# JacobYoung115/VisualSLAM

Hardware: AMD Instinct MI355X
Metric: frames/sec @1080p (Harris + DoG keypoint detection) (higher is better)
Workload: dtype u8

## Files before the change

### visualslam_amd/csrc/kernels_compact.hip.h

```cpp
#pragma once
#include <hip/hip_runtime.h>

#include "kernels_generic.hip.h"
#include "kernels_harris_strip.hip.h"

namespace vslam {

constexpr int CMP_CHUNK = 256;

__device__ __forceinline__ int select64(unsigned long long w, unsigned int k) {
    unsigned int x = (unsigned int)w;
    int pos = 0;
    unsigned int c = __popc(x);
    if (k >= c) k -= c, pos = 32, x = (unsigned int)(w >> 32);
#pragma unroll
    for (int s = 16; s >= 1; s >>= 1) {
        c = __popc(x & ((1u << s) - 1u));
        if (k >= c) k -= c, pos += s, x >>= s;
    }
    return pos;
}

struct HarrisStripEntries {
    static constexpr int WORDS = 4;
    struct Info {
        int row, c0;
    };
    const unsigned long long* flags;
    size_t fframe;
    int rows, cols, nstrips;
    const float* resp;
    size_t rframe;
    vslam_kp* out;
    __device__ size_t count() const { return (size_t)rows * nstrips; }
    __device__ unsigned int load(int f, size_t e, unsigned long long (&w)[4]) const {
        const unsigned long long* F = flags + f * fframe + e * 4;
#pragma unroll
        for (int k = 0; k < 4; ++k) w[k] = F[k];
        return __popcll(w[0]) + __popcll(w[1]) + __popcll(w[2]) + __popcll(w[3]);
    }
    __device__ Info info(int, size_t e) const {
        const int r = (int)((unsigned int)e / (unsigned int)nstrips), strip = (int)((unsigned int)e % (unsigned int)nstrips);
        return Info{r, strip * HS_STRIP_W - 8};
    }
    __device__ void emit(int f, const Info& in, const unsigned long long (&w)[4], unsigned int k, size_t slot) const {
        int l = 0;
#pragma unroll
        for (int s = 32; s >= 1; s >>= 1) {
            const unsigned long long m = (1ull << (l + s)) - 1ull;
            const unsigned int c = __popcll(w[0] & m) + __popcll(w[1] & m) + __popcll(w[2] & m) + __popcll(w[3] & m);
            if (c <= k) l += s;
        }
        const unsigned long long m = (1ull << l) - 1ull;
        k -= __popcll(w[0] & m) + __popcll(w[1] & m) + __popcll(w[2] & m) + __popcll(w[3] & m);
        const unsigned int nib = (unsigned int)((w[0] >> l) & 1ull) | ((unsigned int)((w[1] >> l) & 1ull) << 1) |
                                 ((unsigned int)((w[2] >> l) & 1ull) << 2) | ((unsigned int)((w[3] >> l) & 1ull) << 3);
        unsigned int x = nib;
        for (unsigned int i = 0; i < k; ++i) x &= x - 1;
        const int c = in.c0 + 4 * l + (__ffs((int)x) - 1);
        vslam_kp kp;
        kp.row = in.row;
        kp.col = c;
        kp.response = resp[f * rframe + (size_t)in.row * cols + c];
        out[slot] = kp;
    }
};

struct DogEntries {
    static constexpr int WORDS = 1;
    struct Info {
        int octave, level, i, j0, step;
        unsigned int row_off;
    };
    const unsigned long long* lflags;
    size_t bframe;
    const uint8_t* pyr;
    size_t pframe;
    ExtGeom g;
    int o_begin, o_end;
    vslam_point* out;
    __device__ size_t first() const { return g.bits_off[o_begin]; }
    __device__ size_t count() const {
        return g.bits_off[o_end - 1] + (size_t)3 * g.lat_rows[o_end - 1] * g.wpr[o_end - 1] - g.bits_off[o_begin];
    }
    __device__ unsigned int load(int f, size_t e, unsigned long long (&w)[4]) const {
        w[0] = lflags[f * bframe + first() + e];
        return __popcll(w[0]);
    }
    __device__ Info info(int, size_t e) const {
        const size_t wi = first() + e;
        int o = o_begin;
        while (o + 1 < o_end && wi >= g.bits_off[o + 1]) ++o;
        const unsigned int wl = (unsigned int)(wi - g.bits_off[o]);
        const unsigned int wpr = g.wpr[o], lr = g.lat_rows[o];
        const int level = (int)(wl / (lr * wpr)) + 1;
        const int li = (int)((wl / wpr) % lr), lj0 = (int)(wl % wpr) * 64;
        const size_t P = (size_t)g.rows[o] * g.pitch[o];
        const int i = g.pad + li * g.window;
        return Info{o, level, i, g.pad + lj0 * g.window, g.window,
                    (unsigned int)(g.oct_off[o] + (size_t)(VSLAM_NUM_LEVELS + level) * P + (size_t)(i - g.pad) * g.pitch[o])};
    }
    __device__ void emit(int f, const Info& in, const unsigned long long (&w)[4], unsigned int k, size_t slot) const {
        const int j = in.j0 + select64(w[0], k) * in.step;
        vslam_point pt;
        pt.row = in.i;
        pt.col = j;
        pt.value = pyr[f * pframe + in.row_off + (j - g.pad)];
        if (g.localize) {
            const int o = in.octave;
            const size_t P = (size_t)g.rows[o] * g.pitch[o];
            const uint8_t* dog = pyr + f * pframe + g.oct_off[o] + (size_t)VSLAM_NUM_LEVELS * P;
            int d_x, d_y, d_s, nv;
            dog_differences(dog, P, g.rows[o], g.cols[o], g.pitch[o], g.pad, in.level, in.i, j, d_x, d_y, d_s);
            feature_point_localization(d_x, d_y, d_s, pt.value, nv, g.loc_lut);
            pt.value = nv;
        }
        pt.padding = g.pad;
        pt.octave = in.octave;
        pt.level = in.level;
        out[slot] = pt;
    }
};

struct OrientEntries {
    static constexpr int WORDS = 1;
    struct Info {
        int row, col, octave, level;
    };
    const unsigned long long* masks;
    const vslam_point* kps;
    size_t n;
    vslam_point* out;
    __device__ size_t count() const { return n; }
    __device__ unsigned int load(int, size_t e, unsigned long long (&w)[4]) const {
        w[0] = masks[e];
        return __popcll(w[0]);
    }
    __device__ Info info(int, size_t e) const {
        const vslam_point kp = kps[e];
        return Info{kp.row, kp.col, kp.octave, kp.level};
    }
    __device__ void emit(int, const Info& in, const unsigned long long (&w)[4], unsigned int k, size_t slot) const {
        vslam_point pt;
        pt.row = in.row;
        pt.col = in.col;
        pt.value = select64(w[0], k) * 10;
        pt.padding = 0;
        pt.octave = in.octave;
        pt.level = in.level;
        out[slot] = pt;
    }
};

struct SurvivorEntries {
    static constexpr int WORDS = 1;
    struct Info {
        unsigned int first;
    };
    const unsigned long long* flags;
    size_t fwords;
    unsigned int* surv;
    __device__ size_t count() const { return fwords; }
    __device__ unsigned int load(int f, size_t e, unsigned long long (&w)[4]) const {
        w[0] = flags[f * fwords + e];
        return __popcll(w[0]);
    }
    __device__ Info info(int, size_t e) const { return Info{(unsigned int)(e * 64)}; }
    __device__ void emit(int, const Info& in, const unsigned long long (&w)[4], unsigned int k, size_t slot) const {
        surv[slot] = in.first + (unsigned int)select64(w[0], k);
    }
};

struct OrientBatchEntries {
    static constexpr int WORDS = 1;
    struct Info {
        int row, col, octave, level;
    };
    const unsigned long long* masks;
    const unsigned int* surv;
    const unsigned int* scounts;
    unsigned int scap;
    const vslam_point* pts;
    unsigned int pcap;
    vslam_point* out;
    __device__ size_t count() const { return scap; }
    __device__ unsigned int load(int f, size_t e, unsigned long long (&w)[4]) const {
        w[0] = e < min(scounts[f], scap) ? masks[(size_t)f * scap + e] : 0ull;
        return __popcll(w[0]);
    }
    __device__ Info info(int f, size_t e) const {
        const vslam_point kp = pts[(size_t)f * pcap + surv[(size_t)f * scap + e]];
        return Info{kp.row, kp.col, kp.octave, kp.level};
    }
    __device__ void emit(int, const Info& in, const unsigned long long (&w)[4], unsigned int k, size_t slot) const {
        vslam_point pt;
        pt.row = in.row;
        pt.col = in.col;
        pt.value = select64(w[0], k) * 10;
        pt.padding = 0;
        pt.octave = in.octave;
        pt.level = in.level;
        out[slot] = pt;
    }
};

struct MatchEntries {
    static constexpr int WORDS = 1;
    struct Info {
        unsigned int first;
    };
    const unsigned long long* flags;
    size_t fwords;
    const vslam_nn2* nn;
    unsigned int qcap;
    vslam_match* out;
    __device__ size_t count() const { return fwords; }
    __device__ unsigned int load(int f, size_t e, unsigned long long (&w)[4]) const {
        w[0] = flags[f * fwords + e];
        return __popcll(w[0]);
    }
    __device__ Info info(int, size_t e) const { return Info{(unsigned int)(e * 64)}; }
    __device__ void emit(int f, const Info& in, const unsigned long long (&w)[4], unsigned int k, size_t slot) const {
        const unsigned int q = in.first + (unsigned int)select64(w[0], k);
        const vslam_nn2 r = nn[(size_t)f * qcap + q];
        vslam_match m;
        m.query = (int)q;
        m.train = r.index;
        m.dist2 = r.dist2;
        out[slot] = m;
    }
};

struct EpipolarEntries {
    static constexpr int WORDS = 1;
    struct Info {
        unsigned int first;
    };
    const unsigned long long* flags;
    size_t fwords;
    const vslam_match* matches;
    const unsigned int* counts;
    unsigned int mcap;
    vslam_match* out;
    __device__ size_t count() const { return fwords; }
    __device__ unsigned int load(int f, size_t e, unsigned long long (&w)[4]) const {
        w[0] = e * 64 < min(counts[f], mcap) ? flags[f * fwords + e] : 0ull;
        return __popcll(w[0]);
    }
    __device__ Info info(int, size_t e) const { return Info{(unsigned int)(e * 64)}; }
    __device__ void emit(int f, const Info& in, const unsigned long long (&w)[4], unsigned int k, size_t slot) const {
        out[slot] = matches[(size_t)f * mcap + in.first + (unsigned int)select64(w[0], k)];
    }
};

__device__ __forceinline__ unsigned int block_excl_scan_256(unsigned int v, unsigned int* wsum, unsigned int& total) {
    const int lane = threadIdx.x & 63, wave = threadIdx.x >> 6;
    unsigned int inc = v;
    for (int off = 1; off < 64; off <<= 1) {
        const unsigned int t = __shfl_up(inc, off);
        if (lane >= off) inc += t;
    }
    if (lane == 63) wsum[wave] = inc;
    __syncthreads();
    unsigned int base = 0, tot = 0;
#pragma unroll
    for (int w = 0; w < 4; ++w) {
        const unsigned int s = wsum[w];
        if (w < wave) base += s;
        tot += s;
    }
    total = tot;
    return base + inc - v;
}

template <class E>
__global__ __launch_bounds__(256) void k_flag_count(const E ent, unsigned int* __restrict__ chunk_tot, int nchunks) {
    __shared__ unsigned int wsum[4];
    const int f = blockIdx.z;
    const size_t e = (size_t)blockIdx.x * CMP_CHUNK + threadIdx.x;
    unsigned long long w[4] = {0, 0, 0, 0};
    const unsigned int cnt = e < ent.count() ? ent.load(f, e, w) : 0u;
    unsigned int total;
    block_excl_scan_256(cnt, wsum, total);
    if (threadIdx.x == 0) chunk_tot[(size_t)f * nchunks + blockIdx.x] = total;
}

__global__ __launch_bounds__(256) void k_chunk_scan(unsigned int* __restrict__ chunk_tot, int nchunks,
                                                     unsigned int* __restrict__ counts, int append) {
    __shared__ unsigned int wsum[4];
    const int f = blockIdx.x;
    unsigned int* T = chunk_tot + (size_t)f * nchunks;
    unsigned int running = append ? counts[f] : 0u;
    for (int base = 0; base < nchunks; base += 256) {
        const int i = base + threadIdx.x;
        const unsigned int v = i < nchunks ? T[i] : 0u;
        unsigned int total;
        const unsigned int ex = block_excl_scan_256(v, wsum, total);
        if (i < nchunks) T[i] = running + ex;
        running += total;
        __syncthreads();
    }
    if (threadIdx.x == 0) counts[f] = running;
}

template <class E>
__global__ __launch_bounds__(256) void k_flag_scatter(const E ent, const unsigned int* __restrict__ chunk_off, int nchunks,
                                                       unsigned int cap) {
    __shared__ unsigned int wsum[4];
    __shared__ unsigned int s_ex[CMP_CHUNK];
    __shared__ unsigned long long s_w[E::WORDS][CMP_CHUNK];
    __shared__ typename E::Info s_info[CMP_CHUNK];
    const int f = blockIdx.z, t = threadIdx.x;
    const size_t e = (size_t)blockIdx.x * CMP_CHUNK + t;
    unsigned long long w[4] = {0, 0, 0, 0};
    const unsigned int cnt = e < ent.count() ? ent.load(f, e, w) : 0u;
    unsigned int total;
    s_ex[t] = block_excl_scan_256(cnt, wsum, total);
#pragma unroll
    for (int k = 0; k < E::WORDS; ++k) s_w[k][t] = w[k];
    if (cnt) s_info[t] = ent.info(f, e);
    __syncthreads();
    const unsigned int base = chunk_off[(size_t)f * nchunks + blockIdx.x];
    if (base >= cap) return;
    for (unsigned int r = t; r < total; r += CMP_CHUNK) {
        if (base + r >= cap) break;
        int lo = 0;
#pragma unroll
        for (int s = CMP_CHUNK / 2; s >= 1; s >>= 1)
            if (s_ex[lo + s] <= r) lo += s;
        unsigned long long we[4] = {0, 0, 0, 0};
#pragma unroll
        for (int k = 0; k < E::WORDS; ++k) we[k] = s_w[k][lo];
        ent.emit(f, s_info[lo], we, r - s_ex[lo], (size_t)f * cap + base + r);
    }
}

__global__ __launch_bounds__(256) void k_pack_offsets(const unsigned int* __restrict__ counts, unsigned int cap, int n,
                                                       unsigned long long* __restrict__ offsets) {
    __shared__ unsigned long long sc[256];
    const int t = threadIdx.x;
    unsigned long long running = 0;
    for (int base = 0; base < n; base += 256) {
        const int i = base + t;
        const unsigned long long v = i < n ? (unsigned long long)min(counts[i], cap) : 0ull;
        sc[t] = v;
        __syncthreads();
        for (int off = 1; off < 256; off <<= 1) {
            const unsigned long long a = t >= off ? sc[t - off] : 0ull;
            __syncthreads();
            sc[t] += a;
            __syncthreads();
        }
        if (i < n) offsets[i] = running + sc[t] - v;
        running += sc[255];
        __syncthreads();
    }
    if (t == 0) offsets[n] = running;
}

__global__ __launch_bounds__(256) void k_pack_copy(const unsigned int* __restrict__ lists, unsigned int rec_dw, unsigned int cap,
                                                    const unsigned int* __restrict__ counts,
                                                    const unsigned long long* __restrict__ offsets,
                                                    unsigned int* __restrict__ packed, unsigned long long packed_dw) {
    const int f = blockIdx.z;
    const unsigned long long ndw = (unsigned long long)min(counts[f], cap) * rec_dw;
    const unsigned int* src = lists + (size_t)f * cap * rec_dw;
    const unsigned long long d0 = offsets[f] * rec_dw;
    for (unsigned long long i = (unsigned long long)blockIdx.x * 256 + threadIdx.x; i < ndw; i += (unsigned long long)gridDim.x * 256)
        if (d0 + i < packed_dw) packed[d0 + i] = src[i];
}

__global__ __launch_bounds__(256) void k_pack_points16(const int2* __restrict__ lists, unsigned int cap, const unsigned int* __restrict__ counts,
                                                        const unsigned long long* __restrict__ offsets, uint4* __restrict__ packed,
                                                        unsigned long long packed_recs) {
    const int f = blockIdx.z;
    const unsigned int nrec = min(counts[f], cap);
    const int2* src = lists + (size_t)f * cap * 3;
    const unsigned long long d0 = offsets[f];
    for (unsigned int i = blockIdx.x * 256 + threadIdx.x; i < nrec; i += gridDim.x * 256) {
        const int2 a = src[3 * (size_t)i], b = src[3 * (size_t)i + 1], c = src[3 * (size_t)i + 2];
        if (d0 + i < packed_recs)
            packed[d0 + i] = make_uint4((unsigned int)a.x, (unsigned int)a.y, (unsigned int)b.x,
                                        ((unsigned int)c.y & 0xffu) | (((unsigned int)c.x & 0xffu) << 8) | (((unsigned int)b.y & 0xffffu) << 16));
    }
}

__global__ __launch_bounds__(256) void k_count_totals(const unsigned int* __restrict__ a, const unsigned int* __restrict__ b, int n,
                                                       unsigned long long* __restrict__ totals) {
    __shared__ unsigned long long sa[4], sb[4];
    unsigned long long ta = 0, tb = 0;
    for (int i = threadIdx.x; i < n; i += 256) {
        if (a) ta += a[i];
        if (b) tb += b[i];
    }
    for (int off = 32; off >= 1; off >>= 1) {
        ta += __shfl_down(ta, off);
        tb += __shfl_down(tb, off);
    }
    if ((threadIdx.x & 63) == 0) sa[threadIdx.x >> 6] = ta, sb[threadIdx.x >> 6] = tb;
    __syncthreads();
    if (threadIdx.x == 0) {
        totals[0] = sa[0] + sa[1] + sa[2] + sa[3];
        totals[1] = sb[0] + sb[1] + sb[2] + sb[3];
    }
}

}
```

### visualslam_amd/csrc/kernels_harris_strip.hip.h

```cpp
#pragma once
#include <hip/hip_runtime.h>

#include <type_traits>

#include "kernels_generic.hip.h"
#include "vslam_harris_launch.h"

namespace vslam {

typedef short s2_t __attribute__((ext_vector_type(2)));

__device__ __forceinline__ uint32_t pk_sub_i16(uint32_t a, uint32_t b) {
    return __builtin_bit_cast(uint32_t, (s2_t)(__builtin_bit_cast(s2_t, a) - __builtin_bit_cast(s2_t, b)));
}
struct HarrisStripArgs {
    const uint8_t* img;
    size_t frame;
    int rows, cols;
    float k;
    float* resp;
    uint8_t* mask;
    float* nms2;
    unsigned long long* flags;
    size_t fframe;
    int nstrips, seg;
    uint8_t* dump;
};

__device__ __forceinline__ uint32_t dpp_left(uint32_t v) { return (uint32_t)__builtin_amdgcn_mov_dpp((int)v, 0x138, 0xf, 0xf, true); }
__device__ __forceinline__ uint32_t dpp_right(uint32_t v) { return (uint32_t)__builtin_amdgcn_mov_dpp((int)v, 0x130, 0xf, 0xf, true); }
__device__ __forceinline__ float dpp_left_f(float v) { return __uint_as_float(dpp_left(__float_as_uint(v))); }
__device__ __forceinline__ float dpp_right_f(float v) { return __uint_as_float(dpp_right(__float_as_uint(v))); }
__device__ __forceinline__ float max3f(float a, float b, float c) { return __builtin_fmaxf(__builtin_fmaxf(a, b), c); }

__device__ __forceinline__ uint32_t umax3(uint32_t a, uint32_t b, uint32_t c) { return max(max(a, b), c); }

template <bool ANYW, bool EDGE>
__device__ __forceinline__ void harris_strip_rows(const HarrisStripArgs& a, const int lane, const int strip, const int y_begin,
                                                  const int y_end) {
    const int rows = a.rows, cols = a.cols;
    const size_t N = (size_t)rows * cols;
    const uint8_t* src = a.img + blockIdx.z * a.frame;
    const int x0 = strip * HS_STRIP_W + 4 * (lane - 2);
    const bool lane_in = x0 >= 0 && x0 < cols;
    const bool lane_full = x0 >= 0 && x0 + 4 <= cols;
    const bool lane_out = lane >= 2 && lane < 62 && lane_in;
    const bool left_edge = x0 == 0, right_edge = x0 + 4 == cols;
    const int jedge = ANYW && lane_in && !lane_full ? cols - x0 : 0;
    bool inter[4];
#pragma unroll
    for (int k = 0; k < 4; ++k) inter[k] = lane_out && x0 + k >= 2 && x0 + k < cols - 2;
    unsigned long long inter_m[4];
#pragma unroll
    for (int k = 0; k < 4; ++k) inter_m[k] = __builtin_amdgcn_ballot_w64(inter[k]);

    auto load_row = [&](int t) -> uint32_t {
        const uint8_t* row = src + (size_t)reflect101(t, rows) * cols;
        if (!EDGE) {
            uint32_t w;
            const uint32_t roff = __builtin_amdgcn_readfirstlane((uint32_t)reflect101(t, rows) * (uint32_t)cols);
            __builtin_memcpy(&w, src + roff + (uint32_t)x0, 4);
            return w;
        }
        if (ANYW ? lane_full : lane_in) {
            uint32_t w;
            __builtin_memcpy(&w, row + x0, 4);
            return w;
        }
        return (uint32_t)row[reflect101(x0, cols)] | ((uint32_t)row[reflect101(x0 + 1, cols)] << 8) |
               ((uint32_t)row[reflect101(x0 + 2, cols)] << 16) | ((uint32_t)row[reflect101(x0 + 3, cols)] << 24);
    };

    uint32_t e1 = 0, o1 = 0, e2 = 0, o2 = 0;
    uint32_t be2 = 0, bo2 = 0, be1 = 0, bo1 = 0;
    int PA[3][4] = {}, PB[3][4] = {};
    uint32_t h3a[4] = {}, h3b[4] = {};
    uint32_t h4a[4] = {}, h4b[4] = {}, h4c[4] = {};
    uint32_t Ry[4] = {}, Cy[4] = {}, nby[4] = {};

    const int t_begin = y_begin - 5, t_end = y_end + 3;
    uint32_t nxt0 = load_row(t_begin), nxt1 = load_row(t_begin + 1);
    auto trip = [&](auto steady_tag, const int t0) {
    constexpr bool STEADY = decltype(steady_tag)::value;
#pragma unroll
    for (int u = 0; u < 6; ++u) {
        const int t = t0 + u;
        const uint32_t raw = nxt0;
        nxt0 = nxt1;
        if constexpr (STEADY) {
            const uint32_t roff = __builtin_amdgcn_readfirstlane((uint32_t)(t + 2) * (uint32_t)cols);
            __builtin_memcpy(&nxt1, src + roff + (uint32_t)x0, 4);
        } else {
            nxt1 = load_row(t + 2);
        }

        const uint32_t e3 = raw & 0x00ff00ffu, o3 = (raw >> 8) & 0x00ff00ffu;
        const uint32_t ve = e1 + e3 + (e2 << 1), vo = o1 + o3 + (o2 << 1);
        const uint32_t lvo = dpp_left(vo), rve = dpp_right(ve);
        const uint32_t he = __builtin_amdgcn_alignbit(vo, lvo, 16) + vo + (ve << 1) + 0x00080008u;
        const uint32_t ho = __builtin_amdgcn_alignbit(rve, ve, 16) + ve + (vo << 1) + 0x00080008u;
        const uint32_t be0 = pk_lshr_u16(he, 4), bo0 = pk_lshr_u16(ho, 4);
        e1 = e2, o1 = o2, e2 = e3, o2 = o3;

        const uint32_t lbo = dpp_left(bo1), rbe = dpp_right(be1);
        const uint32_t ixe = pk_sub_i16(bo1, __builtin_amdgcn_alignbit(bo1, lbo, 16));
        const uint32_t ixo = pk_sub_i16(__builtin_amdgcn_alignbit(rbe, be1, 16), be1);
        const uint32_t iye = pk_sub_i16(be0, be2), iyo = pk_sub_i16(bo0, bo2);
        be2 = be1, bo2 = bo1, be1 = be0, bo1 = bo0;
        int ix[4], iy[4];
        ix[0] = (int)(short)(ixe & 0xffff), ix[2] = (int)ixe >> 16, ix[1] = (int)(short)(ixo & 0xffff), ix[3] = (int)ixo >> 16;
        iy[0] = (int)(short)(iye & 0xffff), iy[2] = (int)iye >> 16, iy[1] = (int)(short)(iyo & 0xffff), iy[3] = (int)iyo >> 16;
        int PC[3][4];
#pragma unroll
        for (int k = 0; k < 4; ++k) {
            PC[0][k] = ix[k] * ix[k];
            PC[1][k] = iy[k] * iy[k];
            PC[2][k] = ix[k] * iy[k];
        }

        const int b = t - 3;
        uint32_t Rb[4];
        if (STEADY || (b >= 0 && b < rows)) {
            int V[3][4];
            if (!STEADY && (b - 1 < 0 || b + 1 >= rows)) {
                asm volatile("");
                const bool top_rep = b - 1 < 0, bot_rep = b + 1 >= rows;
#pragma unroll
                for (int c = 0; c < 3; ++c)
#pragma unroll
                    for (int k = 0; k < 4; ++k) V[c][k] = (top_rep ? PB[c][k] : PA[c][k]) + PB[c][k] + (bot_rep ? PB[c][k] : PC[c][k]);
            } else {
#pragma unroll
                for (int c = 0; c < 3; ++c)
#pragma unroll
                    for (int k = 0; k < 4; ++k) V[c][k] = PA[c][k] + PB[c][k] + PC[c][k];
            }
            int S[3][4];
#pragma unroll
            for (int c = 0; c < 3; ++c) {
                int vm1 = (int)dpp_left((uint32_t)V[c][3]), v4 = (int)dpp_right((uint32_t)V[c][0]);
                if (EDGE) {
                    if (ANYW) {
#pragma unroll
                        for (int j = 1; j <= 3; ++j)
                            if (jedge == j) V[c][j] = V[c][j - 1];
                    }
                    vm1 = left_edge ? V[c][0] : vm1;
                    v4 = right_edge ? V[c][3] : v4;
                }
                const int a01 = V[c][0] + V[c][1], a23 = V[c][2] + V[c][3];
                S[c][0] = a01 + vm1;
                S[c][1] = a01 + V[c][2];
                S[c][2] = a23 + V[c][1];
                S[c][3] = a23 + v4;
            }
#pragma unroll
            for (int k = 0; k < 4; ++k) {
                const double det_d = __builtin_fma(-(double)S[2][k], (double)S[2][k], (double)S[0][k] * (double)S[1][k]);
                const float det = (float)det_d;
                const float tr = (float)(S[0][k] + S[1][k]);
                const float trtr = tr * tr;
                const float ktr = a.k * trtr;
                Rb[k] = __float_as_uint(__builtin_fmaxf(det - ktr, 0.0f));
            }
            if (EDGE) {
#pragma unroll
                for (int k = 0; k < 4; ++k) {
                    const bool px_in = ANYW ? (lane_in && (lane_full || k < jedge)) : lane_in;
                    Rb[k] = px_in ? Rb[k] : 0u;
                }
            }
        } else {
#pragma unroll
            for (int k = 0; k < 4; ++k) Rb[k] = 0u;
        }
#pragma unroll
        for (int c = 0; c < 3; ++c)
#pragma unroll
            for (int k = 0; k < 4; ++k) PA[c][k] = PB[c][k], PB[c][k] = PC[c][k];

        uint32_t h3n[4], h4n[4], nbn[4], Cb[4];
        {
            const uint32_t l2 = dpp_left(Rb[2]), l3 = dpp_left(Rb[3]), r0 = dpp_right(Rb[0]);
            const uint32_t m01 = max(Rb[0], Rb[1]), m23 = max(Rb[2], Rb[3]);
            h4n[0] = umax3(l2, l3, m01);
            h4n[1] = umax3(l3, m01, Rb[2]);
            h4n[2] = max(m01, m23);
            h4n[3] = umax3(Rb[1], m23, r0);
        }
#pragma unroll
        for (int k = 0; k < 4; ++k) Cb[k] = __float_as_uint(__builtin_rintf(__uint_as_float(min(Rb[k], 0x437f0000u))));
        if (__builtin_amdgcn_ballot_w64(h4n[2] >= 0x4f000000u)) {
            asm volatile("");
#pragma unroll
            for (int k = 0; k < 4; ++k) Cb[k] = Rb[k] < 0x4f000000u ? Cb[k] : 0u;
        }
        nbn[0] = max(dpp_left(Cb[3]), Cb[1]);
        nbn[1] = max(Cb[0], Cb[2]);
        nbn[2] = max(Cb[1], Cb[3]);
        nbn[3] = max(dpp_right(Cb[0]), Cb[2]);
#pragma unroll
        for (int k = 0; k < 4; ++k) h3n[k] = max(nbn[k], Cb[k]);

        const int y = t - 4;
        if (STEADY || (y >= y_begin && y < y_end)) {
            uint32_t mword = 0;
#pragma unroll
            for (int k = 0; k < 4; ++k) {
                const uint32_t mx = umax3(h3a[k], h3n[k], nby[k]);
                mword |= Cy[k] > mx ? 0xffu << (8 * k) : 0u;
            }
            uint32_t n2[4] = {0u, 0u, 0u, 0u};
            unsigned long long kpw[4] = {0ull, 0ull, 0ull, 0ull};
            if (STEADY || (y >= 2 && y < rows - 2)) {
#pragma unroll
                for (int k = 0; k < 4; ++k) {
                    const uint32_t w4 = max(umax3(h4a[k], h4b[k], h4c[k]), h4n[k]);
                    const bool pass = inter[k] && Ry[k] >= w4;
                    n2[k] = pass ? w4 : 0u;
                    kpw[k] = __builtin_amdgcn_ballot_w64(Ry[k] >= w4) & __builtin_amdgcn_ballot_w64(w4 - 0x437d8000u < 0x4f000000u - 0x437d8000u) & inter_m[k];
                }
            }
            if constexpr (STEADY) {
                const size_t off = blockIdx.z * N + __builtin_amdgcn_readfirstlane((uint32_t)y * (uint32_t)cols) + x0;
                const ptrdiff_t dr = lane_out ? reinterpret_cast<const uint8_t*>(a.resp + off) - a.dump : 0;
                const ptrdiff_t dm = lane_out ? (a.mask + off) - a.dump : 16;
                *reinterpret_cast<float4*>(a.dump + dr) = make_float4(__uint_as_float(Ry[0]), __uint_as_float(Ry[1]), __uint_as_float(Ry[2]), __uint_as_float(Ry[3]));
                *reinterpret_cast<uint32_t*>(a.dump + dm) = mword;
                unsigned long long* F = a.flags + blockIdx.z * a.fframe + ((size_t)y * a.nstrips + strip) * 4;
                F[0] = kpw[0], F[1] = kpw[1], F[2] = kpw[2], F[3] = kpw[3];
            } else {
            if (lane_out) {
                const size_t off = blockIdx.z * N + __builtin_amdgcn_readfirstlane((uint32_t)y * (uint32_t)cols) + x0;
                const float4 rv = make_float4(__uint_as_float(Ry[0]), __uint_as_float(Ry[1]), __uint_as_float(Ry[2]), __uint_as_float(Ry[3]));
                const float4 nv = make_float4(__uint_as_float(n2[0]), __uint_as_float(n2[1]), __uint_as_float(n2[2]), __uint_as_float(n2[3]));
                if (!ANYW) {
                    if (a.resp) *reinterpret_cast<float4*>(a.resp + off) = rv;
                    if (a.mask) *reinterpret_cast<uint32_t*>(a.mask + off) = mword;
                    if (a.nms2) *reinterpret_cast<float4*>(a.nms2 + off) = nv;
                } else if (!EDGE || lane_full) {
                    if (a.resp) __builtin_memcpy(a.resp + off, &rv, 16);
                    if (a.mask) __builtin_memcpy(a.mask + off, &mword, 4);
                    if (a.nms2) __builtin_memcpy(a.nms2 + off, &nv, 16);
                } else {
#pragma unroll
                    for (int k = 0; k < 3; ++k)
                        if (k < jedge) {
                            if (a.resp) a.resp[off + k] = __uint_as_float(Ry[k]);
                            if (a.mask) a.mask[off + k] = (uint8_t)(mword >> (8 * k));
                            if (a.nms2) a.nms2[off + k] = __uint_as_float(n2[k]);
                        }
                }
            }
            if (a.flags && lane == 0) {
                unsigned long long* F = a.flags + blockIdx.z * a.fframe + ((size_t)y * a.nstrips + strip) * 4;
                F[0] = kpw[0], F[1] = kpw[1], F[2] = kpw[2], F[3] = kpw[3];
            }
            }
        }
#pragma unroll
        for (int k = 0; k < 4; ++k) {
            h3a[k] = h3b[k], h3b[k] = h3n[k];
            h4a[k] = h4b[k], h4b[k] = h4c[k], h4c[k] = h4n[k];
            Ry[k] = Rb[k], Cy[k] = Cb[k], nby[k] = nbn[k];
        }
    }
    };
    const bool fast_ok = !EDGE && !ANYW && a.resp && a.mask && a.flags && !a.nms2 && a.dump;
    const int y_lo = max(y_begin, 2), y_hi = min(y_end, rows - 2);
    int t0 = t_begin;
    const int t_hi = min(y_hi - 1, rows - 7);
    for (; t0 <= t_end && !(fast_ok && t0 - 4 >= y_lo && t0 < t_hi && t0 + 2 >= 0); t0 += 6) trip(std::false_type{}, t0);
    if constexpr (!EDGE && !ANYW) {
        if (fast_ok && t0 <= t_end && t0 < t_hi) {
            trip(std::true_type{}, t0);
            t0 += 6;
        }
        for (; fast_ok && t0 <= t_end && t0 < t_hi; t0 += 6) trip(std::true_type{}, t0);
    }
    for (; t0 <= t_end; t0 += 6) trip(std::false_type{}, t0);
}

template <bool ANYW>
__global__ __launch_bounds__(256) __attribute__((amdgpu_waves_per_eu(4, 4))) void k_harris_strip(const HarrisStripArgs a) {
    const int lane = threadIdx.x & 63;
    const int wid = __builtin_amdgcn_readfirstlane(blockIdx.x * 4 + (threadIdx.x >> 6));
    const int nseg = (a.rows + a.seg - 1) / a.seg;
    if (wid >= a.nstrips * nseg) return;
    const int strip = wid % a.nstrips, sgi = wid / a.nstrips;
    const int y_begin = sgi * a.seg, y_end = min(y_begin + a.seg, a.rows);
    const bool edge_strip = strip == 0 || (strip + 1) * HS_STRIP_W + 8 > a.cols;
    if (edge_strip)
        harris_strip_rows<ANYW, true>(a, lane, strip, y_begin, y_end);
    else
        harris_strip_rows<ANYW, false>(a, lane, strip, y_begin, y_end);
}

}
```

Baseline: 15100.

## Transpose Harris flag bitmaps on load and simplify steady-state stores

The compaction loader now transposes the four per-strip flag words into column-ordered bits. Emit can then locate the k-th keypoint with a word select plus select64, instead of a 6-step binary search over four masked popcounts and a serial nibble loop. In the Harris strip kernel's steady loop, store pointers for response, mask and flags are computed once and advanced by increments each row, rather than recomputed per row. The keypoint ballot is cheapened by folding the range check into umax3, with the overflow check applied only when a wrap was seen. The added bit-spreading work in load and the deferred wrap flag add register pressure and some risk of subtle edge-case mismatches.

```diff
diff --git a/visualslam_amd/csrc/kernels_compact.hip.h b/visualslam_amd/csrc/kernels_compact.hip.h
--- a/visualslam_amd/csrc/kernels_compact.hip.h
+++ b/visualslam_amd/csrc/kernels_compact.hip.h
@@ -19,6 +19,12 @@
         if (k >= c) k -= c, pos += s, x >>= s;
     }
     return pos;
+}
+
+__device__ __forceinline__ unsigned int spread8_by4(unsigned int b) {
+    b = (b | (b << 12)) & 0x000f000fu;
+    b = (b | (b << 6)) & 0x03030303u;
+    return (b | (b << 3)) & 0x11111111u;
 }
 
 struct HarrisStripEntries {
@@ -35,29 +41,34 @@
     __device__ size_t count() const { return (size_t)rows * nstrips; }
     __device__ unsigned int load(int f, size_t e, unsigned long long (&w)[4]) const {
         const unsigned long long* F = flags + f * fframe + e * 4;
-#pragma unroll
-        for (int k = 0; k < 4; ++k) w[k] = F[k];
-        return __popcll(w[0]) + __popcll(w[1]) + __popcll(w[2]) + __popcll(w[3]);
+        unsigned int lo[4], hi[4];
+#pragma unroll
+        for (int k = 0; k < 4; ++k) lo[k] = (unsigned int)F[k], hi[k] = (unsigned int)(F[k] >> 32);
+#pragma unroll
+        for (int j = 0; j < 4; ++j) {
+            unsigned int d[2];
+#pragma unroll
+            for (int h = 0; h < 2; ++h) {
+                const int m = 2 * j + h;
+                d[h] = 0;
+#pragma unroll
+                for (int k = 0; k < 4; ++k) d[h] |= spread8_by4(((m < 4 ? lo[k] : hi[k]) >> (8 * (m & 3))) & 0xffu) << k;
+            }
+            w[j] = (unsigned long long)d[0] | ((unsigned long long)d[1] << 32);
+        }
+        return __popc(lo[0]) + __popc(hi[0]) + __popc(lo[1]) + __popc(hi[1]) + __popc(lo[2]) + __popc(hi[2]) + __popc(lo[3]) + __popc(hi[3]);
     }
     __device__ Info info(int, size_t e) const {
         const int r = (int)((unsigned int)e / (unsigned int)nstrips), strip = (int)((unsigned int)e % (unsigned int)nstrips);
         return Info{r, strip * HS_STRIP_W - 8};
     }
     __device__ void emit(int f, const Info& in, const unsigned long long (&w)[4], unsigned int k, size_t slot) const {
-        int l = 0;
-#pragma unroll
-        for (int s = 32; s >= 1; s >>= 1) {
-            const unsigned long long m = (1ull << (l + s)) - 1ull;
-            const unsigned int c = __popcll(w[0] & m) + __popcll(w[1] & m) + __popcll(w[2] & m) + __popcll(w[3] & m);
-            if (c <= k) l += s;
-        }
-        const unsigned long long m = (1ull << l) - 1ull;
-        k -= __popcll(w[0] & m) + __popcll(w[1] & m) + __popcll(w[2] & m) + __popcll(w[3] & m);
-        const unsigned int nib = (unsigned int)((w[0] >> l) & 1ull) | ((unsigned int)((w[1] >> l) & 1ull) << 1) |
-                                 ((unsigned int)((w[2] >> l) & 1ull) << 2) | ((unsigned int)((w[3] >> l) & 1ull) << 3);
-        unsigned int x = nib;
-        for (unsigned int i = 0; i < k; ++i) x &= x - 1;
-        const int c = in.c0 + 4 * l + (__ffs((int)x) - 1);
+        const unsigned int c0 = __popcll(w[0]), c1 = c0 + __popcll(w[1]), c2 = c1 + __popcll(w[2]);
+        const bool g0 = k >= c0, g1 = k >= c1, g2 = k >= c2;
+        const unsigned long long ws = g1 ? (g2 ? w[3] : w[2]) : (g0 ? w[1] : w[0]);
+        k -= g1 ? (g2 ? c2 : c1) : (g0 ? c0 : 0u);
+        const int j = (int)g0 + (int)g1 + (int)g2;
+        const int c = in.c0 + 64 * j + select64(ws, k);
         vslam_kp kp;
         kp.row = in.row;
         kp.col = c;
diff --git a/visualslam_amd/csrc/kernels_harris_strip.hip.h b/visualslam_amd/csrc/kernels_harris_strip.hip.h
--- a/visualslam_amd/csrc/kernels_harris_strip.hip.h
+++ b/visualslam_amd/csrc/kernels_harris_strip.hip.h
@@ -80,6 +80,16 @@
 
     const int t_begin = y_begin - 5, t_end = y_end + 3;
     uint32_t nxt0 = load_row(t_begin), nxt1 = load_row(t_begin + 1);
+    bool wrap_y = false;
+    uint8_t *st_resp = nullptr, *st_mask = nullptr;
+    unsigned long long* st_flags = nullptr;
+    const unsigned long long st_step = lane_out ? (unsigned long long)cols : 0ull;
+    auto steady_begin = [&](const int y) {
+        const size_t off = blockIdx.z * N + (size_t)y * cols + x0;
+        st_resp = lane_out ? reinterpret_cast<uint8_t*>(a.resp + off) : a.dump;
+        st_mask = lane_out ? a.mask + off : a.dump + 16;
+        st_flags = a.flags + blockIdx.z * a.fframe + ((size_t)y * a.nstrips + strip) * 4;
+    };
     auto trip = [&](auto steady_tag, const int t0) {
     constexpr bool STEADY = decltype(steady_tag)::value;
 #pragma unroll
@@ -190,7 +200,8 @@
         }
 #pragma unroll
         for (int k = 0; k < 4; ++k) Cb[k] = __float_as_uint(__builtin_rintf(__uint_as_float(min(Rb[k], 0x437f0000u))));
-        if (__builtin_amdgcn_ballot_w64(h4n[2] >= 0x4f000000u)) {
+        const bool wrap_b = __builtin_amdgcn_ballot_w64(h4n[2] >= 0x4f000000u) != 0;
+        if (wrap_b) {
             asm volatile("");
 #pragma unroll
             for (int k = 0; k < 4; ++k) Cb[k] = Rb[k] < 0x4f000000u ? Cb[k] : 0u;
@@ -215,6 +226,11 @@
             if (STEADY || (y >= 2 && y < rows - 2)) {
 #pragma unroll
                 for (int k = 0; k < 4; ++k) {
+                    if constexpr (STEADY) {
+                        const uint32_t w4lo = umax3(umax3(h4a[k], h4b[k], h4c[k]), h4n[k], 0x437d8000u);
+                        kpw[k] = __builtin_amdgcn_ballot_w64(Ry[k] >= w4lo) & inter_m[k];
+                        continue;
+                    }
                     const uint32_t w4 = max(umax3(h4a[k], h4b[k], h4c[k]), h4n[k]);
                     const bool pass = inter[k] && Ry[k] >= w4;
                     n2[k] = pass ? w4 : 0u;
@@ -222,13 +238,15 @@
                 }
             }
             if constexpr (STEADY) {
-                const size_t off = blockIdx.z * N + __builtin_amdgcn_readfirstlane((uint32_t)y * (uint32_t)cols) + x0;
-                const ptrdiff_t dr = lane_out ? reinterpret_cast<const uint8_t*>(a.resp + off) - a.dump : 0;
-                const ptrdiff_t dm = lane_out ? (a.mask + off) - a.dump : 16;
-                *reinterpret_cast<float4*>(a.dump + dr) = make_float4(__uint_as_float(Ry[0]), __uint_as_float(Ry[1]), __uint_as_float(Ry[2]), __uint_as_float(Ry[3]));
-                *reinterpret_cast<uint32_t*>(a.dump + dm) = mword;
-                unsigned long long* F = a.flags + blockIdx.z * a.fframe + ((size_t)y * a.nstrips + strip) * 4;
-                F[0] = kpw[0], F[1] = kpw[1], F[2] = kpw[2], F[3] = kpw[3];
+                if (wrap_y) {
+                    asm volatile("");
+#pragma unroll
+                    for (int k = 0; k < 4; ++k) kpw[k] &= __builtin_amdgcn_ballot_w64(Ry[k] < 0x4f000000u);
+                }
+                *reinterpret_cast<float4*>(st_resp) = make_float4(__uint_as_float(Ry[0]), __uint_as_float(Ry[1]), __uint_as_float(Ry[2]), __uint_as_float(Ry[3]));
+                *reinterpret_cast<uint32_t*>(st_mask) = mword;
+                st_flags[0] = kpw[0], st_flags[1] = kpw[1], st_flags[2] = kpw[2], st_flags[3] = kpw[3];
+                st_resp += st_step << 2, st_mask += st_step, st_flags += 4 * a.nstrips;
             } else {
             if (lane_out) {
                 const size_t off = blockIdx.z * N + __builtin_amdgcn_readfirstlane((uint32_t)y * (uint32_t)cols) + x0;
@@ -264,6 +282,7 @@
             h4a[k] = h4b[k], h4b[k] = h4c[k], h4c[k] = h4n[k];
             Ry[k] = Rb[k], Cy[k] = Cb[k], nby[k] = nbn[k];
         }
+        wrap_y = wrap_b;
     }
     };
     const bool fast_ok = !EDGE && !ANYW && a.resp && a.mask && a.flags && !a.nms2 && a.dump;
@@ -273,6 +292,7 @@
     for (; t0 <= t_end && !(fast_ok && t0 - 4 >= y_lo && t0 < t_hi && t0 + 2 >= 0); t0 += 6) trip(std::false_type{}, t0);
     if constexpr (!EDGE && !ANYW) {
         if (fast_ok && t0 <= t_end && t0 < t_hi) {
+            steady_begin(t0 - 4);
             trip(std::true_type{}, t0);
             t0 += 6;
         }
```

Result: no change. 15080 (-0.1%).
